# szcompressor/sz

Measured on AMD Instinct MI355X. Metric: compression GB/s (input), 512^3 float32 ABS 1e-4, higher is better.
Workload: dtype f32

## Files before the change

### sz_amd/csrc/szh_fittile.h

```cpp
#pragma once

namespace szh_ft {
constexpr int BMAX = 7;
constexpr int LPR = 1;
template <class T> struct shape {
    static constexpr int VT = 16 / (int)sizeof(T);
    static constexpr int SEGB = sizeof(T) == 4 ? 32 : 16;
    static constexpr int WIDTH = SEGB * BMAX + 2 * VT;
    static constexpr int PITCH = WIDTH + VT;
    static constexpr int BUF = BMAX * PITCH;
    static_assert((WIDTH + VT - 1) / VT <= 64 * LPR && PITCH % VT == 0, "row pieces per lane");
};
template <class T> inline bool applies(const szh_geom3 &G, const void *base)
{
    if (G.ndim != 3) return false;
    if (G.g0.early > BMAX || G.g1.early > BMAX || G.g2.early > BMAX) return false;
    if (G.g0.count < 2 || G.g1.count < 2 || G.g2.count < 2) return false;
    if ((G.g2.count % shape<T>::VT) != 0 || ((uintptr_t)base & 15) != 0) return false;
    return (double)G.g0.num * G.g1.num * ((G.g2.num + shape<T>::SEGB - 1) / shape<T>::SEGB) < 2.0e9;
}
}

template <class T>
__global__ __launch_bounds__(64) void k_fit_tile(szh_geom3 G, const T *__restrict__ data, T *coef, uint8_t *blk_lor, T noise, int use_mean, T mean, u64 *minmax, int nseg)
{
    using namespace szh_ft;
    typedef shape<T> S;
    constexpr int VT = S::VT;
    __shared__ __attribute__((aligned(16))) T buf[2][S::BUF];
    const int lane = (int)threadIdx.x;
    const int col = (int)(blockIdx.x / (unsigned)nseg), segi = (int)(blockIdx.x - (unsigned)col * (unsigned)nseg);
    const int b0 = col / G.g1.num, b1 = col - b0 * G.g1.num;
    const int s0 = szh_blk_size(G.g0, b0), s1 = szh_blk_size(G.g1, b1), o0 = szh_blk_start(G.g0, b0), o1 = szh_blk_start(G.g1, b1);
    const int bkbeg = segi * S::SEGB, bkend = bkbeg + S::SEGB < G.g2.num ? bkbeg + S::SEGB : G.g2.num;
    const int kbeg = szh_blk_start(G.g2, bkbeg), kend = bkend < G.g2.num ? szh_blk_start(G.g2, bkend) : G.g2.count;
    const int ka = kbeg / VT * VT, kb = (kend + VT - 1) / VT * VT, nvec = (kb - ka) / VT;
    const int b2 = bkbeg + lane;
    const bool has = b2 < bkend;
    const int s2 = has ? szh_blk_size(G.g2, b2) : 1, k0 = has ? szh_blk_start(G.g2, b2) - ka : 0;
    int bs = s0 < s1 ? s0 : s1; if (s2 < bs) bs = s2;

    const T qnan = (T)__builtin_nanf("");
    T vmin = qnan, vmax = qnan;
    uint4 pf[BMAX][LPR];
    auto fetch = [&](int i) {
#pragma unroll
        for (int j = 0; j < BMAX; ++j)
#pragma unroll
            for (int q = 0; q < LPR; ++q) {
                const int v = lane + 64 * q;
                pf[j][q] = uint4{0u, 0u, 0u, 0u};
                if (j < s1 && v < nvec) pf[j][q] = *reinterpret_cast<const uint4 *>(data + (int64_t)(o0 + i) * G.d0 + (int64_t)(o1 + j) * G.d1 + ka + v * VT);
            }
    };
    auto place = [&](int w) {
#pragma unroll
        for (int j = 0; j < BMAX; ++j)
#pragma unroll
            for (int q = 0; q < LPR; ++q) {
                const int v = lane + 64 * q;
                if (j < s1 && v < nvec) {
                    *reinterpret_cast<uint4 *>(&buf[w][j * S::PITCH + v * VT]) = pf[j][q];
                    T x[VT]; __builtin_memcpy(x, &pf[j][q], 16);
                    const int e_lo = kbeg - (ka + v * VT), e_hi = kend - (ka + v * VT);
#pragma unroll
                    for (int e = 0; e < VT; ++e) {
                        const T xv = (e >= e_lo && e < e_hi) ? x[e] : qnan;
                        vmin = sizeof(T) == 8 ? (T)__builtin_fmin((double)vmin, (double)xv) : (T)__builtin_fminf((float)vmin, (float)xv);
                        vmax = sizeof(T) == 8 ? (T)__builtin_fmax((double)vmax, (double)xv) : (T)__builtin_fmaxf((float)vmax, (float)xv);
                    }
                }
            }
    };
    fetch(0);
    T fx = 0, fy = 0, fz = 0, f = 0, err_sz = 0;
    T xs[4 * (BMAX - 1)];
#pragma unroll
    for (int e = 0; e < 4 * (BMAX - 1); ++e) xs[e] = 0;
#pragma unroll
    for (int i = 0; i < BMAX; ++i) {
        if (i >= s0) break;
        const int w = i & 1;
        place(w);
        __syncthreads();
        if (i + 1 < s0) fetch(i + 1);
        if (has) {
            const T *P = &buf[w][k0], *Q = &buf[w ^ 1][k0];
            T sum_x = 0;
#pragma unroll
            for (int j = 0; j < BMAX; ++j) {
                if (j < s1) {
                    T row[BMAX];
#pragma unroll
                    for (int k = 0; k < BMAX; ++k) row[k] = k < s2 ? P[j * S::PITCH + k] : (T)0;
                    T sum_y = 0;
#pragma unroll
                    for (int k = 0; k < BMAX; ++k) if (k < s2) { const T c = row[k]; sum_y += c; fz += c * (T)k; }
                    fy += sum_y * (T)j;
                    sum_x += sum_y;
                }
            }
            fx += sum_x * (T)i;
            f += sum_x;
            if (i >= 1 && i < bs) {
                const int bmi = bs - i;
#pragma unroll
                for (int q = 0; q < 4; ++q) {
                    const int j = (q & 2) ? bmi : i, k = (q & 1) ? bmi : i;
                    const T x = P[j * S::PITCH + k];
                    const T psz = P[j * S::PITCH + k - 1] + P[(j - 1) * S::PITCH + k] + Q[j * S::PITCH + k] - P[(j - 1) * S::PITCH + k - 1] - Q[j * S::PITCH + k - 1]
                                  - Q[(j - 1) * S::PITCH + k] + Q[(j - 1) * S::PITCH + k - 1];
                    const T e1 = szh_abs(psz - x) + noise;
                    if (use_mean) { const T e2 = szh_abs(mean - x); err_sz += (e1 < e2 ? e1 : e2); }
                    else err_sz += e1;
                    xs[(i - 1) * 4 + q] = x;
                }
            }
        }
        __syncthreads();
    }
    if (has) {
        const T coeff = (T)(1.0 / (double)((int64_t)s0 * s1 * s2));
        const T a = ((T)2 * fx / (T)(s0 - 1) - f) * (T)6 * coeff / (T)(s0 + 1);
        const T b = ((T)2 * fy / (T)(s1 - 1) - f) * (T)6 * coeff / (T)(s1 + 1);
        const T c = ((T)2 * fz / (T)(s2 - 1) - f) * (T)6 * coeff / (T)(s2 + 1);
        const T d = f * coeff - ((T)(s0 - 1) * a / (T)2 + (T)(s1 - 1) * b / (T)2 + (T)(s2 - 1) * c / (T)2);
        T err_reg = 0;
#pragma unroll
        for (int i = 1; i < BMAX; ++i) {
            if (i < bs) {
                const int bmi = bs - i;
#pragma unroll
                for (int q = 0; q < 4; ++q) {
                    const int j = (q & 2) ? bmi : i, k = (q & 1) ? bmi : i;
                    const T preg = a * (T)i + b * (T)j + c * (T)k + d;
                    err_reg += szh_abs(preg - xs[(i - 1) * 4 + q]);
                }
            }
        }
        const int64_t blk = ((int64_t)b0 * G.g1.num + b1) * G.g2.num + b2;
        coef[blk] = a; coef[G.nblocks + blk] = b; coef[2 * G.nblocks + blk] = c; coef[3 * G.nblocks + blk] = d;
        blk_lor[blk] = err_reg < err_sz ? 0 : 1;
    }
    u64 lmin = vmin == vmin ? ord_enc(vmin) : ~0ull, lmax = vmax == vmax ? ord_enc(vmax) : 0ull;
    lmin = wave_min_u64(lmin); lmax = wave_max_u64(lmax);
    if (lane == 0) {
        if (lmin < *(volatile u64 *)&minmax[0]) atomicMin(&minmax[0], lmin);
        if (lmax > *(volatile u64 *)&minmax[1]) atomicMax(&minmax[1], lmax);
    }
}
```

### sz_amd/csrc/szhip_kernels.h

```cpp
#pragma once
#include <hip/hip_runtime.h>
#include "szh_core.h"
#include "szh_pencil.h"
#include "szh_bufio.h"

typedef unsigned long long u64;

#ifdef SZH_HIPSIM
#define SZH_DYN_SMEM(name) char *name = hipsim_dyn_smem()
#else
#define SZH_DYN_SMEM(name) extern __shared__ __attribute__((aligned(16))) char name[]
#endif

__device__ __forceinline__ u64 ord_enc(float v)
{
    unsigned u = __float_as_uint(v);
    u = (u & 0x80000000u) ? ~u : (u | 0x80000000u);
    return (u64)u;
}
__device__ __forceinline__ u64 ord_enc(double v)
{
    u64 u = (u64)__double_as_longlong(v);
    u = (u & 0x8000000000000000ull) ? ~u : (u | 0x8000000000000000ull);
    return u;
// ... 211 lines not shown
        } else if (w == NP) szh_tile_store<T, B>(a, TI, TJ, L);
        else szh_tile_fill<T, B>(a, TI, TJ, L);
        if (!a.persist) break;
    }
}

template <class T> struct GlobAcc {
    const T *p; int64_t d0, d1;
    __device__ T operator()(int i, int j, int k) const { return p[i * d0 + j * d1 + k]; }
    __device__ T operator()(int j, int k) const { return p[j * d1 + k]; }
};

template <class T>
__global__ __launch_bounds__(256) void k_fit_select(szh_geom3 G, const T *__restrict__ data, T *coef, uint8_t *blk_lor,
                                                    T noise, int use_mean, T mean, u64 *minmax)
{
    __shared__ u64 red[8];
    const int lane = threadIdx.x & 63, wid = threadIdx.x >> 6;
    const int64_t b = (int64_t)blockIdx.x * 256 + threadIdx.x;
    u64 lmin = ~0ull, lmax = 0ull;
    if (b < G.nblocks) {
        const int nb2 = G.g2.num, nb1 = G.g1.num;
        const int b2 = (int)(b % nb2);
        const int64_t c = b / nb2;
        const int b1 = (int)(c % nb1), b0 = (int)(c / nb1);
        const int s0 = szh_blk_size(G.g0, b0), s1 = szh_blk_size(G.g1, b1), s2 = szh_blk_size(G.g2, b2);
        const GlobAcc<T> A{data + (int64_t)szh_blk_start(G.g0, b0) * G.d0 + (int64_t)szh_blk_start(G.g1, b1) * G.d1 + szh_blk_start(G.g2, b2),
                           G.d0, G.d1};
        T c4[4];
        auto range = [&](T v) { const u64 oe = ord_enc(v); const bool num = v == v; lmin = num && oe < lmin ? oe : lmin; lmax = num && oe > lmax ? oe : lmax; };
        int reg;
        if (G.ndim == 2) {
            c4[0] = 0;
            szh_fit_block_2d<T>(A, s1, s2, c4 + 1, range);
            reg = szh_select_block_2d<T>(A, s1, s2, c4 + 1, noise);
        } else {
            szh_fit_block<T>(A, s0, s1, s2, c4, range);
            reg = szh_select_block<T>(A, s0, s1, s2, c4, noise, use_mean, mean);
        }
        for (int e = 0; e < 4; ++e) coef[(int64_t)e * G.nblocks + b] = c4[e];
        blk_lor[b] = reg ? 0 : 1;
    }
    lmin = wave_min_u64(lmin); lmax = wave_max_u64(lmax);
    if (lane == 0) { red[wid] = lmin; red[4 + wid] = lmax; }
    __syncthreads();
    if (threadIdx.x == 0) {
        u64 mn = red[0], mx = red[4];
        for (int w = 1; w < 4; ++w) { mn = red[w] < mn ? red[w] : mn; mx = red[4 + w] > mx ? red[4 + w] : mx; }
        atomicMin(&minmax[0], mn); atomicMax(&minmax[1], mx);
    }
}

template <class T>
__global__ __launch_bounds__(256) void k_minmax(const T *__restrict__ data, int64_t n, u64 *minmax)
{
    __shared__ u64 red[8];
    u64 lmin = ~0ull, lmax = 0ull;
    for (int64_t i = (int64_t)blockIdx.x * 256 + threadIdx.x; i < n; i += (int64_t)gridDim.x * 256) {
        const T v = data[i]; const u64 e = ord_enc(v); const bool num = v == v;
        lmin = num && e < lmin ? e : lmin; lmax = num && e > lmax ? e : lmax;
    }
    lmin = wave_min_u64(lmin); lmax = wave_max_u64(lmax);
    if ((threadIdx.x & 63) == 0) { red[threadIdx.x >> 6] = lmin; red[4 + (threadIdx.x >> 6)] = lmax; }
    __syncthreads();
    if (threadIdx.x == 0) {
        u64 mn = red[0], mx = red[4];
        for (int w = 1; w < 4; ++w) { mn = red[w] < mn ? red[w] : mn; mx = red[4 + w] > mx ? red[4 + w] : mx; }
        atomicMin(&minmax[0], mn); atomicMax(&minmax[1], mx);
    }
}

template <class T>
__global__ __launch_bounds__(256) void k_gather_mean(const T *__restrict__ data, szh_meanwalk w, int64_t count, T *out)
{
    const int64_t m = (int64_t)blockIdx.x * 256 + threadIdx.x;
    if (m < count) out[m] = data[szh_meanwalk_pos(w, m)];
}

#define SZH_LDS_RADIUS_BINS 4096
template <class T, bool FREQ>
__device__ __forceinline__ void sample_body(szh_geom3 G, const T *__restrict__ data, int64_t nrows, int sd, double ebD, T mean,
                                            unsigned max_radius, unsigned *radius_hist, unsigned *freq_hist, u64 *within)
{
    __shared__ unsigned sh_r[SZH_LDS_RADIUS_BINS];
    __shared__ unsigned sh_f[FREQ ? 8192 : 1];
    for (int i = threadIdx.x; i < SZH_LDS_RADIUS_BINS; i += 256) sh_r[i] = 0;
    if (FREQ) for (int i = threadIdx.x; i < 8192; i += 256) sh_f[i] = 0;
    __syncthreads();
    const int64_t rpp = G.g1.count - 1, r2 = G.g2.count;
    const bool two_d = G.ndim == 2;
    unsigned w = 0;
    for (int64_t ridx = (int64_t)blockIdx.x * 256 + threadIdx.x; ridx < nrows; ridx += (int64_t)gridDim.x * 256) {
        const int64_t n1 = two_d ? 0 : ridx / rpp + 1, n2 = two_d ? ridx + 1 : ridx - (n1 - 1) * rpp + 1;
        const int64_t c0 = two_d ? szh_sample_col0_2d(n2, sd) : sd - ((n1 + n2) % sd);
        const int64_t origin = n1 * G.d0 + n2 * r2;
        for (int64_t m = 0;; ++m) {
            const int64_t col = c0 + m * sd;
            if (m > 0 && col >= r2) break;
            const int64_t pos = origin + col;
            if (pos >= G.n) break;
            unsigned ri; int fi, we;
            szh_sample_point<T>(data, pos, r2, two_d ? 0 : G.d0, ebD, mean, max_radius, &ri, &fi, &we);
            if (ri < SZH_LDS_RADIUS_BINS) atomicAdd(&sh_r[ri], 1u); else atomicAdd(&radius_hist[ri], 1u);
            if (FREQ) atomicAdd(&sh_f[fi], 1u);
            w += (unsigned)we;
        }
    }
    w = wave_sum_u32(w);
    if ((threadIdx.x & 63) == 0 && w) atomicAdd(within, (u64)w);
    __syncthreads();
    for (int i = threadIdx.x; i < SZH_LDS_RADIUS_BINS; i += 256) if (sh_r[i]) atomicAdd(&radius_hist[i], sh_r[i]);
    if (FREQ) for (int i = threadIdx.x; i < 8192; i += 256) if (sh_f[i]) atomicAdd(&freq_hist[i], sh_f[i]);
}
template <class T, bool FREQ>
__global__ __launch_bounds__(256) void k_sample(szh_geom3 G, const T *__restrict__ data, int64_t nrows, int sd, double ebD, T mean,
                                                unsigned max_radius, unsigned *radius_hist, unsigned *freq_hist, u64 *within)
{
    sample_body<T, FREQ>(G, data, nrows, sd, ebD, mean, max_radius, radius_hist, freq_hist, within);
}
template <class T, bool FREQ>
__global__ void k_sample_walk(szh_geom3 G, const T *__restrict__ data, int sd, double ebD, T mean, unsigned max_radius, unsigned *radius_hist,
                              unsigned *freq_hist, u64 *within)
{
    if (threadIdx.x != 0 || blockIdx.x != 0) return;
    const int64_t r3 = G.g2.count, r2 = G.g1.count, r23 = r2 * r3, len = G.n;
    int64_t oc = sd - 2, n1 = 1, n2 = 1, pos = r23 + r3 + oc;
    u64 w = 0;
    while (pos < len) {
        unsigned ri; int fi, we;
        szh_sample_point<T>(data, pos, r3, r23, ebD, mean, max_radius, &ri, &fi, &we);
        atomicAdd(&radius_hist[ri], 1u);
        if (FREQ) atomicAdd(&freq_hist[fi], 1u);
        w += (unsigned)we;
        oc += sd;
        if (oc >= r3) {
            n2++;
            if (n2 == r2) { n1++; n2 = 1; pos += r3; }
            const int64_t oc2 = (n1 + n2) % sd;
            pos += (r3 + sd - oc) + (sd - oc2);
            oc = sd - oc2;
            if (oc == 0) oc++;
        } else pos += sd;
    }
    if (w) atomicAdd(within, w);
}

template <class T>
__device__ __forceinline__ void sample_view_body(const unsigned tid, szh_geom3 G, const T *data, int64_t p0, int64_t p1, int64_t nrows, int sd, double ebD,
                                                 unsigned max_radius, unsigned *radius_hist, u64 *within)
{
    __shared__ unsigned sh_r[SZH_LDS_RADIUS_BINS];
    for (int i = tid; i < SZH_LDS_RADIUS_BINS; i += 256) sh_r[i] = 0;
    __syncthreads();
    const int64_t rpp = G.g1.count - 1, r2 = G.g2.count;
    unsigned w = 0;
    for (int64_t ridx = (int64_t)blockIdx.x * 256 + tid; ridx < nrows; ridx += (int64_t)gridDim.x * 256) {
        const int64_t n1 = ridx / rpp + 1, n2 = ridx - (n1 - 1) * rpp + 1;
        const int64_t c0 = sd - ((n1 + n2) % sd);
        const int64_t origin = n1 * G.d0 + n2 * r2;
        for (int64_t m = 0;; ++m) {
            const int64_t col = c0 + m * sd;
            if (m > 0 && col >= r2) break;
            const int64_t pos = origin + col;
            if (pos >= G.n) break;
            unsigned ri; int fi, we;
            if (col < r2) szh_sample_point<T>(data, n1 * p0 + n2 * p1 + col, p1, p0, ebD, (T)0, max_radius, &ri, &fi, &we);
            else szh_sample_point_view<T>(data, pos, r2, G.d0, p0, p1, ebD, max_radius, &ri, &we);
            if (ri < SZH_LDS_RADIUS_BINS) atomicAdd(&sh_r[ri], 1u); else atomicAdd(&radius_hist[ri], 1u);
            w += (unsigned)we;
        }
    }
    w = wave_sum_u32(w);
    if ((tid & 63) == 0 && w) atomicAdd(within, (u64)w);
    __syncthreads();
    for (int i = tid; i < SZH_LDS_RADIUS_BINS; i += 256) if (sh_r[i]) atomicAdd(&radius_hist[i], sh_r[i]);
}
template <class T>
__global__ __launch_bounds__(256) void k_sample_view(szh_geom3 G, const T *__restrict__ data, int64_t p0, int64_t p1, int64_t nrows, int sd, double ebD,
                                                     unsigned max_radius, unsigned *radius_hist, u64 *within)
{
    __shared__ unsigned sh_r[SZH_LDS_RADIUS_BINS];
    for (int i = threadIdx.x; i < SZH_LDS_RADIUS_BINS; i += 256) sh_r[i] = 0;
    __syncthreads();
    const int64_t rpp = G.g1.count - 1, r2 = G.g2.count;
    unsigned w = 0;
    for (int64_t ridx = (int64_t)blockIdx.x * 256 + threadIdx.x; ridx < nrows; ridx += (int64_t)gridDim.x * 256) {
        const int64_t n1 = ridx / rpp + 1, n2 = ridx - (n1 - 1) * rpp + 1;
        const int64_t c0 = sd - ((n1 + n2) % sd);
        const int64_t origin = n1 * G.d0 + n2 * r2;
        for (int64_t m = 0;; ++m) {
            const int64_t col = c0 + m * sd;
            if (m > 0 && col >= r2) break;
            const int64_t pos = origin + col;
            if (pos >= G.n) break;
            unsigned ri; int fi, we;
// ... 1157 lines not shown
```

### sz_amd/csrc/szhip_sz21.inc

```
static bool book_declines(unsigned rec_status, unsigned long long plan_status, int test_switch) { return rec_status != 0 || plan_status != 0 || test_switch != 0; }

struct sz21_plan {
    bool use_beam = false;
    bool segenc = false;
    bool seghist = false;
    bool dev_book = false;
    bool sliced = false;
    int slices_req = 1;
    int se_vw = 1, se_segb = 0, se_nseg = 0, se_nrmax = szh_se::NR; size_t se_tile = 0;
    int sh_rshift = 0;
    bool revise(unsigned enc_maxlen) { if (!segenc || enc_maxlen <= 32) return false; segenc = false; seghist = false; return true; }
};
template <class T>
sz21_plan sz21_make_plan(const szhip_ctx *ctx, const szh_geom3 &G, unsigned intervals, size_t reg_count, bool beam_ok, bool overlap, bool feed, size_t meta_len)
{
    sz21_plan P;
    const int64_t n = G.n;
    P.use_beam = !overlap && beam_ok;
    const int segenc_sw = tune_int("SZ_HIP_SEGENC", 1);
    P.segenc = G.ndim == 3 && segenc_sw != 0 && (!feed || segenc_sw == 2);
    P.se_vw = (G.g2.count % 8) == 0 ? 8 : ((G.g2.count % 4) == 0 ? 4 : 1);
    if (P.segenc) {
        bool ok = intervals < 65536 && (double)n < 4.0e9;
        if ((int64_t)G.g0.late * G.g1.late * G.g2.late < 32) ok = false;
        const size_t fixed = ((size_t)intervals + 1) * 8 + 16 + szh_se::seg_window_words(G, 32) * 4 + 64;
        const size_t lds_cap = (size_t)63 * 1024, want = (size_t)std::max(4, tune_int("SZ_HIP_SEG_TILE_KB", 14)) * 1024;
        if (ok && fixed + szh_se::seg_tile_bytes(G, 1, P.se_vw) > lds_cap) ok = false;
        if (ok) {
            const size_t budget = std::min(lds_cap - fixed, std::max(want, szh_se::seg_tile_bytes(G, 1, P.se_vw)));
            int sb = 1;
            while (sb < G.g2.num && szh_se::seg_tile_bytes(G, sb + 1, P.se_vw) <= budget && szh_se::seg_pieces_per_thread(G, sb + 1, P.se_vw) <= (size_t)szh_se::PF) ++sb;
            sb = (G.g2.num + (G.g2.num + sb - 1) / sb - 1) / ((G.g2.num + sb - 1) / sb);
            if (const int f = tune_int("SZ_HIP_SEG_SEGB", 0)) sb = std::max(1, std::min(f, sb));
            P.se_segb = sb;
            P.se_nseg = (G.g2.num + sb - 1) / sb;
            P.se_tile = szh_se::seg_tile_bytes(G, sb, P.se_vw);
            const int rows_typ = (2 * G.g0.split > G.g0.num ? G.g0.early : G.g0.late) * (2 * G.g1.split > G.g1.num ? G.g1.early : G.g1.late);
            const int runs_typ = std::max(1, sb * rows_typ), rounds_typ = (runs_typ + 256 * szh_se::NR - 1) / (256 * szh_se::NR);
            P.se_nrmax = std::max(1, std::min(szh_se::NR, (runs_typ + 256 * rounds_typ - 1) / (256 * rounds_typ)));
            if ((double)G.g0.num * G.g1.num >= 2.0e9) ok = false;
        }
        P.segenc = ok;
    }
    P.seghist = P.segenc && intervals <= SZH_COL_HBINS && tune_int("SZ_HIP_SEGHIST", 1) != 0;
    if (P.seghist) P.sh_rshift = hist_rshift(intervals, 4096);
    P.dev_book = P.segenc && reg_count == 0 && !ctx->no_dev_book && tune_int("SZ_HIP_DEV_BOOK", 0) != 0 && G.g0.num * G.g1.num <= 1024 * SZH_COL_SCAN_PER &&
                 tune_int("SZ_HIP_SEG_SCAN1", 1) != 0 && meta_len + 8 + 4 + sizeof(T) + 1 + sizeof(T) <= 3072;
    P.slices_req = tune_int("SZ_HIP_SLICES", ctx->gate ? tune_int("SZ_HIP_SLICES_POOL", 2) : 4);
    P.sliced = P.use_beam && P.slices_req > 1 && !P.seghist;
    return P;
}

template <class T>
struct sz21_call : call_base {
    static constexpr int is_double = sizeof(T) == 8;
    static constexpr int64_t LINE = 128 / (int64_t)sizeof(T);
    const szhip_params *const prm; const unsigned char *meta; const size_t meta_len; const int out_on_device; unsigned char **const out; size_t *const out_size;
    const double eb_in; const T eb;
    const bool two_d;
    const szh_geom3 G; const int ncoef, ncols; const int64_t n, nb;
    const int tp_on = tune_int("SZ_HIP_TIMING", 0); double tp_t[32]; const char *tp_n[32]; int tp_k = 0;
    const T *d_in = nullptr; u64 *sm = nullptr; T *d_coef = nullptr; uint8_t *d_lor = nullptr; uint16_t *d_nat = nullptr, *d_blk = nullptr; unsigned *d_hist = nullptr, *h_hist = nullptr;
    T noise = 0; bool fit_tile = false; int ft_nseg = 0;
    size_t ind_bytes = 0; unsigned char *ind_bits = nullptr; u64 *nreg_h = nullptr, *minmax_h = nullptr;
    unsigned intervals = 0; int use_mean = 0; T mean = 0; size_t reg_count = 0;
    std::vector<unsigned char> meta_own;
    sz21_plan P;
    unsigned *tile_done = nullptr; size_t beam_words = 0;
    int perm_segb = 1, perm_nseg = 1; size_t perm_lds = 0;
    std::vector<szh_se::seg_t> se_segs; std::vector<u64> tab_code; std::vector<uint8_t> tab_len;
    unsigned enc_maxlen = 0; bool enc32 = false; size_t lds_e32 = 0;
    unsigned char *hdr = nullptr; size_t pre_len = 0, sections_total = 0, hdr_len = 0, unpred_bytes = 0, total_len = 0; u64 total_bits = 0, total_unpred = 0;
    u64 h_small[SM_COUNT];
    szhost_coeffs cf;
    size_t sec_len[4] = {0, 0, 0, 0};
    std::vector<std::thread> section_threads;
    std::atomic<int> section_failed{0};
    std::vector<unsigned char> all_reg_keep;
    std::vector<uint32_t> blk_of_rank;
    size_t chain_done[4] = {0, 0, 0, 0};
    size_t chain_avail = 0;
    double chain_t0[4] = {0, 0, 0, 0}, chain_t1[4] = {0, 0, 0, 0};
    bool overlap = false, feed = false, two_pieces = false;
    fed_call_guard fed_guard;
    T *hcoef = nullptr;
    bool pool_busy = false;
    bool cf_own = false;
    sz21_call(szhip_ctx *c, size_t r0, size_t r1, size_t r2, double eb_, const szhip_params *p, const unsigned char *m, size_t ml, int ood, unsigned char **o, size_t *os)
        : call_base(c), prm(p), meta(m), meta_len(ml), out_on_device(ood), out(o), out_size(os), eb_in(eb_), eb((T)eb_), two_d(r0 == 0),
          G(r0 == 0 ? szh_make_geom2((int)r1, (int)r2) : szh_make_geom3((int)r0, (int)r1, (int)r2)), ncoef(r0 == 0 ? 3 : 4), ncols(G.g0.num * G.g1.num), n(G.n), nb(G.nblocks)
    {
        memset(&cf, 0, sizeof(cf));
        S.n_elements = (uint64_t)n; S.n_blocks = (uint64_t)nb;
    }
    ~sz21_call() {
        join_sections();
        if (ctx->chain_pool) ctx->chain_pool->disarm();
        if (cf_own) for (int e = 0; e < 4; ++e) { cf.codes[e] = nullptr; cf.unpred[e] = nullptr; }
        szhost_coeffs_free(&cf);
    }
    void join_sections() {
        for (auto &x : section_threads) if (x.joinable()) x.join();
        if (pool_busy && ctx->chain_pool) { ctx->chain_pool->wait_all(); pool_busy = false; }
    }
    void TP(const char *nm) { if (tp_on && tp_k < 32) { tp_t[tp_k] = now_ms() - t_begin; tp_n[tp_k++] = nm; } }
    void print_trace() const { if (tp_on) { for (int i = 0; i < tp_k; ++i) fprintf(stderr, "%s %.2f | ", tp_n[i], tp_t[i]); fprintf(stderr, "\n"); } }
    bool is_lorenzo(int64_t bb) const { return (ind_bits[bb >> 3] >> (7 - (bb & 7))) & 1; }
    size_t count_lorenzo(int64_t bb, int64_t b_end) const {
        size_t ones = 0;
        for (; bb < b_end && (bb & 7); ++bb) ones += is_lorenzo(bb);
        for (; bb + 64 <= b_end; bb += 64) { uint64_t w8; memcpy(&w8, ind_bits + (bb >> 3), 8); ones += (size_t)__builtin_popcountll(w8); }
        for (; bb < b_end; ++bb) ones += is_lorenzo(bb);
        return ones;
    }
    size_t chains_done() const {
        size_t p = reg_count;
        for (int e = 0; e < ncoef; ++e) { const size_t d = __atomic_load_n(&chain_done[e], __ATOMIC_ACQUIRE); if (d < p) p = d; }
        return p;
    }
    int launch_fit(hipStream_t s_, int um, T mn) {
        if (fit_tile) hipLaunchKernelGGL((k_fit_tile<T>), dim3((unsigned)((int64_t)ncols * ft_nseg)), dim3(64), 0, s_, G, d_in, d_coef, d_lor, noise, um, mn, sm + SM_MINMAX, ft_nseg);
        else hipLaunchKernelGGL((k_fit_select<T>), dim3((unsigned)((nb + 255) / 256)), dim3(256), 0, s_, G, d_in, d_coef, d_lor, noise, um, mn, sm + SM_MINMAX);
        HIPCHK(hipGetLastError());
        return SZHIP_OK;
    }
    int launch_pack_lor(hipStream_t s_) {
        hipLaunchKernelGGL(k_pack_lor, dim3((unsigned)((ind_bytes + 255) / 256)), dim3(256), 0, s_, (const uint8_t *)d_lor, nb, (uint8_t *)ctx->lor_bits.p, sm + SM_NREG);
        HIPCHK(hipGetLastError());
        HIPCHK(hipMemcpyAsync(ind_bits, ctx->lor_bits.p, ind_bytes, hipMemcpyDeviceToHost, s_));
        HIPCHK(hipMemcpyAsync(nreg_h, sm + SM_NREG, 8, hipMemcpyDeviceToHost, s_));
        return SZHIP_OK;
    }
    int stage_and_fit(const void *data, int data_on_device) {
        TRY(stage_input(ctx, data, data_on_device, (size_t)n, &d_in));
        TRY(clear_small(ctx, &sm));
        static const u64 minmax_init[2] = {~0ull, 0ull};
        HIPCHK(hipMemcpyAsync(sm + SM_MINMAX, minmax_init, 16, hipMemcpyHostToDevice, st));
        TRY(ensure(ctx, ctx->coef, (size_t)nb * 4 * sizeof(T)));
        TRY(ensure(ctx, ctx->blk_lor, (size_t)nb));
        d_coef = (T *)ctx->coef.p;
        d_lor = (uint8_t *)ctx->blk_lor.p;
        HIPCHK(hipEventRecord(ctx->ev[0], st));
        TP("ev0");
        HIPCHK(hipEventRecord(ctx->ev_in, st));
        HIPCHK(hipStreamWaitEvent(ctx->stream2, ctx->ev_in, 0));
        noise = (T)((double)eb * (two_d ? 0.81 : 1.22));
        fit_tile = !two_d && szh_ft::applies<T>(G, d_in) && tune_int("SZ_HIP_FIT_TILE", 0) != 0;
        ft_nseg = (G.g2.num + szh_ft::shape<T>::SEGB - 1) / szh_ft::shape<T>::SEGB;
        TRY(launch_fit(ctx->stream2, 0, (T)0));
        ind_bytes = ((size_t)nb + 7) / 8;
        TRY(ensure(ctx, ctx->lor_bits, ind_bytes + 8));
        TRY(ensure_pinned2(ctx, ind_bytes + 32));
        ind_bits = (unsigned char *)ctx->pinned2 + 32;
        nreg_h = (u64 *)ctx->pinned2;
        minmax_h = (u64 *)ctx->pinned2 + 2;
        TRY(launch_pack_lor(ctx->stream2));
        HIPCHK(hipMemcpyAsync(minmax_h, sm + SM_MINMAX, 16, hipMemcpyDeviceToHost, ctx->stream2));
        HIPCHK(hipEventRecord(ctx->ev_fit, ctx->stream2));
        return SZHIP_OK;
    }
    int choose_intervals() {
        intervals = prm->quantization_intervals;
        const unsigned max_radius = prm->max_quant_intervals / 2;
        if (intervals == 0) {
            const int64_t md = (int64_t)(int)std::sqrt((double)n);
            const szh_meanwalk w = two_d ? szh_make_meanwalk(n, INT64_MAX / 2, INT64_MAX / 2, md) : szh_make_meanwalk(n, G.d0, G.g2.count, md);
            int64_t M = 0, M_hi = n / std::max<int64_t>(md - 2, 1) + 2;
            while (szh_meanwalk_pos(w, M_hi) < n) M_hi *= 2;
            while (M < M_hi) { int64_t mid = (M + M_hi) / 2; if (szh_meanwalk_pos(w, mid) >= n) M_hi = mid; else M = mid + 1; }
            TRY(ensure(ctx, ctx->samples, (size_t)M * sizeof(T)));
            TRY(ensure_pinned(ctx, std::max<size_t>((size_t)M * sizeof(T), (size_t)(max_radius + 8192) * 4 + 64)));
            hipLaunchKernelGGL((k_gather_mean<T>), dim3((unsigned)((M + 255) / 256)), dim3(256), 0, st, d_in, w, M, (T *)ctx->samples.p);
            HIPCHK(hipGetLastError());
            HIPCHK(hipMemcpyAsync(ctx->pinned, ctx->samples.p, (size_t)M * sizeof(T), hipMemcpyDeviceToHost, st));
            TP("mean enqueued");
            HIPCHK(hipStreamSynchronize(st));
            TP("mean on host");
            double h0 = now_ms();
            const double smean = szhost_seq_mean(is_double, ctx->pinned, (size_t)M);
            host_ms += now_ms() - h0;
            TRY(ensure(ctx, ctx->hist, (size_t)(max_radius + 8192) * 4 + 64));
            unsigned *d_rh = (unsigned *)ctx->hist.p, *d_fh = d_rh + max_radius;
            HIPCHK(hipMemsetAsync(d_rh, 0, (size_t)(max_radius + 8192) * 4, st));
            const int64_t nrows = szh_sample_row_limit(G, prm->sample_distance);
            if (!two_d && (G.g0.count <= 1 || G.g1.count <= 1)) {
                hipLaunchKernelGGL((k_sample_walk<T, true>), dim3(1), dim3(64), 0, st, G, d_in, prm->sample_distance, (double)eb, (T)smean, max_radius, d_rh, d_fh, sm + SM_WITHIN);
                HIPCHK(hipGetLastError());
            } else if (nrows > 0) {
                int grid = (int)std::min<int64_t>((nrows + 255) / 256, 1024);
                hipLaunchKernelGGL((k_sample<T, true>), dim3(grid), dim3(256), 0, st, G, d_in, nrows, prm->sample_distance, (double)eb, (T)smean, max_radius, d_rh, d_fh, sm + SM_WITHIN);
                HIPCHK(hipGetLastError());
            }
            unsigned *s_hist = (unsigned *)ctx->pinned;
            u64 within = 0;
            HIPCHK(hipMemcpyAsync(s_hist, d_rh, (size_t)(max_radius + 8192) * 4, hipMemcpyDeviceToHost, st));
            HIPCHK(hipMemcpyAsync(&within, sm + SM_WITHIN, 8, hipMemcpyDeviceToHost, st));
            TP("sample enqueued");
            HIPCHK(hipStreamSynchronize(st));
            TP("sample on host");
            h0 = now_ms();
            u64 sample_count = 0;
            for (unsigned i = 0; i < max_radius; ++i) sample_count += s_hist[i];
            szhost_decision dec;
            szhost_decide(is_double, s_hist, max_radius, s_hist + max_radius, sample_count, within, prm->pred_threshold, (double)eb, smean, &dec);
            host_ms += now_ms() - h0;
            intervals = dec.intervals; use_mean = two_d ? 0 : dec.use_mean;
            if (use_mean) {
                T *d_sum = (T *)(sm + SM_MEANSUM);
                hipLaunchKernelGGL((k_mean_seq<T>), dim3(1), dim3(64), 0, st, d_in, n, (T)dec.dense_pos, eb, d_sum, sm + SM_MEANCNT);
                HIPCHK(hipGetLastError());
                T hsum = 0; u64 hcnt = 0;
                HIPCHK(hipMemcpyAsync(&hsum, d_sum, sizeof(T), hipMemcpyDeviceToHost, st));
                HIPCHK(hipMemcpyAsync(&hcnt, sm + SM_MEANCNT, 8, hipMemcpyDeviceToHost, st));
                HIPCHK(hipStreamSynchronize(st));
                if (hcnt > 0) mean = hsum / (T)hcnt;
            }
        }
        if (intervals > 65536 || intervals < 4) FAIL(SZHIP_ERR_UNSUP, "quantization interval count %u outside [4,65536]", intervals);
        S.intervals = intervals; S.use_mean = use_mean;
        return SZHIP_OK;
    }
    int join_fit() {
        HIPCHK(hipStreamWaitEvent(st, ctx->ev_fit, 0));
        if (use_mean) {
            TRY(launch_fit(st, use_mean, mean));
            HIPCHK(hipMemsetAsync(sm + SM_NREG, 0, 8, st));
            TRY(launch_pack_lor(st));
            HIPCHK(hipStreamSynchronize(st));
        } else HIPCHK(hipEventSynchronize(ctx->ev_fit));
        TP("fit joined");
        reg_count = (size_t)*nreg_h;
        S.n_reg_blocks = reg_count;
        if (reg_count == 0 && ctx->chain_pool) ctx->chain_pool->disarm();
        meta_own.assign(meta, meta + meta_len);
        if (prm->flags & SZHIP_RANGE_FROM_DATA) {
            if (meta_len < 4 + 20 + 2 * sizeof(T)) FAIL(SZHIP_ERR_ARG, "parameter bytes too short for a range field");
            const T lo = (T)ord_dec<T>(minmax_h[0]), hi = (T)ord_dec<T>(minmax_h[1]);
            const T range = hi - lo, top = lo + range;
            unsigned char *q = meta_own.data() + 4 + 20;
            if (is_double) { szhost_put_f64be(q, (double)lo); szhost_put_f64be(q + 8, (double)top); }
            else { szhost_put_f32be(q, (float)lo); szhost_put_f32be(q + 4, (float)top); }
            S.vmin = (double)lo; S.vmax = (double)hi;
            if ((double)range <= eb_in) {
                HIPCHK(hipStreamSynchronize(ctx->stream2)); HIPCHK(hipStreamSynchronize(st));
                *out = nullptr; *out_size = 0;
                S.ms_total = now_ms() - t_begin;
                return SZHIP_CONSTANT;
            }
        }
        meta = meta_own.data();
        return SZHIP_OK;
    }
    void make_section(int e) {
        std::vector<uint32_t> h32(65536, 0);
        for (size_t i = 0; i < reg_count; ++i) h32[(size_t)cf.codes[e][i]]++;
        const huff_ptr ch(szhost_huff_build(131072, h32.data(), nullptr, 65536));
        if (!ch) { section_failed = 1; return; }
        const size_t tb = szhost_huff_tree_size(ch.get());
        const size_t enc_cap = (size_t)((ch->total_bits + 7) / 8) + 16;
        if (sizeof(T) + 12 + tb + 8 + enc_cap + 4 + cf.unpred_count[e] * sizeof(T) > ctx->sec_pin_cap[e]) { section_failed = 1; return; }
        unsigned char *const sec0 = ctx->sec_pin[e];
        unsigned char *q = sec0;
        if (is_double) szhost_put_f64be(q, cf.prec[e]); else szhost_put_f32be(q, (float)cf.prec[e]);
        q += sizeof(T);
        szhost_put_u32be(q, 32768); q += 4;
        szhost_put_u32be(q, (uint32_t)tb); q += 4;
        szhost_put_u32be(q, (uint32_t)ch->n_nodes); q += 4;
        szhost_huff_tree_write(ch.get(), q); q += tb;
        const size_t enc = szhost_huff_encode_i32(ch.get(), cf.codes[e], reg_count, q + 8);
        szhost_put_u64be(q, enc); q += 8 + enc;
        szhost_put_u32be(q, (uint32_t)cf.unpred_count[e]); q += 4;
        memcpy(q, cf.unpred[e], cf.unpred_count[e] * sizeof(T)); q += cf.unpred_count[e] * sizeof(T);
        sec_len[e] = (size_t)(q - sec0);
    }
    int prepare_chains() {
        for (int e = 0; e < ncoef; ++e) {
            const size_t bound = sizeof(T) + 12 + (13 * 2 * std::min<size_t>(reg_count, 65536) + 16) + 8 + (8 * reg_count + 16) + 4 + reg_count * sizeof(T) + 64;
            if (ctx->sec_pin_cap[e] < bound) {
                HIPCHK(hipStreamSynchronize(ctx->stream2)); HIPCHK(hipStreamSynchronize(st));
                if (ctx->sec_pin[e]) { HIPCHK(hipHostFree(ctx->sec_pin[e])); ctx->sec_pin[e] = nullptr; ctx->sec_pin_cap[e] = 0; }
                HIPCHK(hipHostMalloc((void **)&ctx->sec_pin[e], bound + bound / 8, hipHostMallocDefault));
                ctx->sec_pin_cap[e] = bound + bound / 8;
            }
        }
        TRY(ensure(ctx, ctx->reg_flags, (size_t)nb * 8));
        TRY(ensure(ctx, ctx->reg_rank, (size_t)nb * 8));
        TRY(ensure(ctx, ctx->coef_compact, reg_count * 4 * sizeof(T)));
        hipLaunchKernelGGL(k_reg_flags, dim3((unsigned)((nb + 255) / 256)), dim3(256), 0, st, (const uint8_t *)d_lor, nb, (u64 *)ctx->reg_flags.p);
        TRY(scan_u64(ctx, (const u64 *)ctx->reg_flags.p, nb, (u64 *)ctx->reg_rank.p, sm + SM_SCRATCH));
        hipLaunchKernelGGL((k_move_coef<T, 0>), dim3((unsigned)((nb + 255) / 256)), dim3(256), 0, st, (const uint8_t *)d_lor, (const u64 *)ctx->reg_rank.p, nb, (int64_t)reg_count, d_coef, (T *)ctx->coef_compact.p);
        HIPCHK(hipGetLastError());
#ifndef SZH_SYNC_LAUNCH
        overlap = !beam_applies<T>(G, d_in, reg_count) && !two_d && !ctx->gate && !ctx->no_chain_overlap && g_compress_calls.load() <= 1;
        if (overlap) { TRY(probe_streams(ctx)); overlap = ctx->streams_independent == 1; }
#endif
        feed = beam_applies<T>(G, d_in, reg_count) && !ctx->gate && !ctx->no_chain_overlap && g_compress_calls.load() <= 1 && tune_int("SZ_HIP_BEAM_FEED", 1) &&
               G.g0.num >= 2 && reg_count >= (size_t)tune_int("SZ_HIP_FEED_MIN_REG", 65536);
#ifndef SZH_SYNC_LAUNCH
        feed = feed && (G.d0 % 128) == 0;
        if (feed) { TRY(probe_streams(ctx)); feed = ctx->streams_independent == 1; }
#endif
        if (feed) feed = fed_guard.try_raise();
        TRY(ensure_pinned3(ctx, reg_count * 4 * sizeof(T) + (overlap ? ((size_t)nb + 64) * 4 * sizeof(T) + 256 : 0)));
        hcoef = (T *)ctx->pinned3;
        return SZHIP_OK;
    }
    int run_chains() {
        chain_avail = reg_count;
        struct AvailAll {
// ... 941 lines not shown
```

Baseline: 377.7.

## Add one-thread-per-block register fit kernel and rework sampling histograms

Adds a new fit kernel, k_fit_wide, where each thread fits one full 3D block from registers. It uses a statically unrolled sliding-window pass over rows and fuses the regression/Lorenzo choice, bit packing and region counting into the same kernel, so the separate pack_lor launch is skipped. It is enabled by default for float. The sampling kernel now packs two 16-bit frequency counters per LDS word with periodic flushes, uses fewer LDS radius bins, and sizes its grid from the CU count. The histogram memset is also moved earlier to overlap with the mean gather. The fully unrolled 49-step body risks high register pressure and low occupancy.

```diff
diff --git a/sz_amd/csrc/szh_fittile.h b/sz_amd/csrc/szh_fittile.h
--- a/sz_amd/csrc/szh_fittile.h
+++ b/sz_amd/csrc/szh_fittile.h
@@ -1,4 +1,5 @@
 #pragma once
+#include <utility>
 
 namespace szh_ft {
 constexpr int BMAX = 7;
@@ -149,3 +150,209 @@
         if (lmax > *(volatile u64 *)&minmax[1]) atomicMax(&minmax[1], lmax);
     }
 }
+
+#ifdef SZH_HIPSIM
+#define SZH_FW_STEP_FENCE() ((void)0)
+#define SZH_FW_PIN(p) ((void)0)
+#else
+#define SZH_FW_STEP_FENCE() __builtin_amdgcn_sched_barrier(0)
+#define SZH_FW_PIN(p) asm volatile("" : "+v"(p))
+#endif
+namespace szh_fw {
+template <class T> struct shape {
+    static constexpr int VT = 16 / (int)sizeof(T);
+    static constexpr int NP = (szh_ft::BMAX + 2 * (VT - 1)) / VT;
+    static constexpr int DEPTH = 1;
+};
+template <class F, int... Is>
+__device__ __forceinline__ void static_steps(F &&f, std::integer_sequence<int, Is...>) { (f(std::integral_constant<int, Is>{}), ...); }
+template <class T>
+__device__ __forceinline__ void block_pass(const szh_geom3 &G, const T *__restrict__ base, int off, int np, int s0, int s1, int s2, T noise, int use_mean, T mean,
+                                           T (&c4)[4], int &reg, T &vmin, T &vmax)
+{
+    constexpr int B = szh_ft::BMAX, VT = shape<T>::VT, NP = shape<T>::NP, D = shape<T>::DEPTH, STEPS = B * B;
+    int bs = s0 < s1 ? s0 : s1; if (s2 < bs) bs = s2;
+    const int d = B - bs;
+    const T qnan = (T)__builtin_nanf("");
+    uint4 buf[D][NP];
+    auto fetch = [&](int slot, int i, int j) {
+        int64_t ro = (int64_t)i * G.d0 + (int64_t)j * G.d1;
+        SZH_FW_PIN(ro);
+        const T *rp = base + ro;
+#pragma unroll
+        for (int q = 0; q < NP; ++q) {
+            const T *p = rp + q * VT;
+            const bool there = i < B - 1 && j < B - 1 ? (q < 2 || q < np) : (i < s0 && j < s1 && q < np);
+            buf[slot][q] = *reinterpret_cast<const uint4 *>(there ? p : base);
+        }
+    };
+    auto pick = [&](const T (&row)[B], int C) -> T {
+        const T a = C >= 0 && C < B ? row[C < 0 ? 0 : (C < B ? C : B - 1)] : (T)0, a1 = C >= 1 && C <= B ? row[C < 1 ? 0 : (C <= B ? C - 1 : B - 1)] : (T)0;
+        return d ? a1 : a;
+    };
+    T fx = 0, fy = 0, fz = 0, f = 0, err_sz = 0, sum_x = 0;
+    T xs[4 * (B - 1)];
+#pragma unroll
+    for (int e = 0; e < 4 * (B - 1); ++e) xs[e] = 0;
+    T Q[4][4], N[4][4], ppc[4], er[4], xv[4];
+#pragma unroll
+    for (int r = 0; r < 4; ++r) {
+        ppc[r] = 0; er[r] = 0; xv[r] = 0;
+#pragma unroll
+        for (int c = 0; c < 4; ++c) { Q[r][c] = 0; N[r][c] = 0; }
+    }
+#pragma unroll
+    for (int t = 0; t < D; ++t) fetch(t, t / B, t % B);
+    static_steps([&](auto tc) {
+        constexpr int t = decltype(tc)::value;
+        constexpr int i = t / B, j = t % B, slot = t % D;
+        T win[NP * VT];
+        __builtin_memcpy(win, buf[slot], sizeof(win));
+        if (t + D < STEPS) fetch(slot, (t + D) / B, (t + D) % B);
+        SZH_FW_STEP_FENCE();
+#pragma unroll
+        for (int s = 1; s < VT; s <<= 1)
+#pragma unroll
+            for (int k = 0; k + s < NP * VT; ++k) win[k] = (off & s) ? win[k + s] : win[k];
+        T row[B];
+#pragma unroll
+        for (int k = 0; k < B; ++k) row[k] = win[k];
+        const bool act = i < s0 && j < s1;
+        if (j == 0) sum_x = 0;
+        T sum_y = 0;
+#pragma unroll
+        for (int k = 0; k < B; ++k) {
+            const bool on = (i < B - 1 && j < B - 1 && k < B - 1) || (act && k < s2);
+            const T c = row[k], cn = on ? c : qnan;
+            sum_y = on ? sum_y + c : sum_y; fz = on ? fz + c * (T)k : fz;
+            vmin = sizeof(T) == 8 ? (T)__builtin_fmin((double)vmin, (double)cn) : (T)__builtin_fminf((float)vmin, (float)cn);
+            vmax = sizeof(T) == 8 ? (T)__builtin_fmax((double)vmax, (double)cn) : (T)__builtin_fmaxf((float)vmax, (float)cn);
+        }
+        const bool act_r = (i < B - 1 && j < B - 1) || act, act_p = i < B - 1 || i < s0;
+        fy = act_r ? fy + sum_y * (T)j : fy; sum_x = act_r ? sum_x + sum_y : sum_x;
+        if (j == B - 1) { fx = act_p ? fx + sum_x * (T)i : fx; f = act_p ? f + sum_x : f; }
+        const int c1 = B - i - d, c0 = c1 - 1;
+        T pc[4];
+        pc[0] = i >= 1 ? row[i >= 1 ? i - 1 : 0] : (T)0; pc[1] = row[i]; pc[2] = pick(row, B - i - 1); pc[3] = pick(row, B - i);
+        if (i + 1 < B) {
+            const T nc[4] = {pc[1], row[i + 1 < B ? i + 1 : B - 1], pick(row, B - i - 2), pc[2]};
+#pragma unroll
+            for (int c = 0; c < 4; ++c) {
+                if (j == i) N[0][c] = nc[c];
+                if (j == i + 1) N[1][c] = nc[c];
+                if (j == B - i - 2 || j == B - i - 3) N[2][c] = (j == c0 - 1) ? nc[c] : N[2][c];
+                if (j == B - i - 1 || j == B - i - 2) N[3][c] = (j == c0) ? nc[c] : N[3][c];
+            }
+        }
+        if (i >= 1 && j >= 1) {
+            auto stencil = [&](const T (&Qj)[4], const T (&Qm)[4], int ck) -> T {
+                const T psz = pc[ck - 1] + ppc[ck] + Qj[ck] - ppc[ck - 1] - Qj[ck - 1] - Qm[ck] + Qm[ck - 1];
+                const T e1 = szh_abs(psz - pc[ck]) + noise;
+                const T e2 = szh_abs(mean - pc[ck]);
+                return (use_mean && e1 >= e2) ? e2 : e1;
+            };
+            if (j == i) { er[0] = stencil(Q[1], Q[0], 1); er[1] = stencil(Q[1], Q[0], 3); xv[0] = pc[1]; xv[1] = pc[3]; }
+            if (j <= B - i && j >= B - i - 1) {
+                const T e2 = stencil(Q[3], Q[2], 1), e3 = stencil(Q[3], Q[2], 3);
+                const bool far = j == c1;
+                er[2] = far ? e2 : er[2]; er[3] = far ? e3 : er[3]; xv[2] = far ? pc[1] : xv[2]; xv[3] = far ? pc[3] : xv[3];
+            }
+        }
+#pragma unroll
+        for (int c = 0; c < 4; ++c) ppc[c] = pc[c];
+        SZH_FW_PIN(fz); SZH_FW_PIN(fy); SZH_FW_PIN(sum_x); SZH_FW_PIN(vmin); SZH_FW_PIN(vmax);
+#pragma unroll
+        for (int c = 0; c < 4; ++c) { SZH_FW_PIN(ppc[c]); SZH_FW_PIN(N[0][c]); SZH_FW_PIN(N[1][c]); SZH_FW_PIN(N[2][c]); SZH_FW_PIN(N[3][c]); SZH_FW_PIN(er[c]); SZH_FW_PIN(xv[c]); }
+        if (j == B - 1) {
+            if (i >= 1) {
+#pragma unroll
+                for (int q = 0; q < 4; ++q) { err_sz = i < bs ? err_sz + er[q] : err_sz; xs[(i >= 1 ? i - 1 : 0) * 4 + q] = xv[q]; }
+            }
+#pragma unroll
+            for (int r = 0; r < 4; ++r)
+#pragma unroll
+                for (int c = 0; c < 4; ++c) Q[r][c] = N[r][c];
+        }
+    }, std::make_integer_sequence<int, STEPS>{});
+    const T coeff = (T)(1.0 / (double)((int64_t)s0 * s1 * s2));
+    const T a = ((T)2 * fx / (T)(s0 - 1) - f) * (T)6 * coeff / (T)(s0 + 1);
+    const T b = ((T)2 * fy / (T)(s1 - 1) - f) * (T)6 * coeff / (T)(s1 + 1);
+    const T c = ((T)2 * fz / (T)(s2 - 1) - f) * (T)6 * coeff / (T)(s2 + 1);
+    const T dd = f * coeff - ((T)(s0 - 1) * a / (T)2 + (T)(s1 - 1) * b / (T)2 + (T)(s2 - 1) * c / (T)2);
+    T err_reg = 0;
+#pragma unroll
+    for (int i = 1; i < B; ++i) {
+        if (i < bs) {
+            const int bmi = bs - i;
+#pragma unroll
+            for (int q = 0; q < 4; ++q) {
+                const int j = (q & 2) ? bmi : i, k = (q & 1) ? bmi : i;
+                const T preg = a * (T)i + b * (T)j + c * (T)k + dd;
+                err_reg += szh_abs(preg - xs[(i - 1) * 4 + q]);
+            }
+        }
+    }
+    c4[0] = a; c4[1] = b; c4[2] = c; c4[3] = dd;
+    reg = err_reg < err_sz ? 1 : 0;
+}
+}
+
+template <class T>
+__global__ __launch_bounds__(256) void k_fit_wide(szh_geom3 G, const T *__restrict__ data, T *coef, uint8_t *blk_lor, uint8_t *bits, u64 *n_reg, T noise, int use_mean,
+                                                  T mean, u64 *minmax)
+{
+    constexpr int VT = szh_fw::shape<T>::VT;
+    __shared__ u64 red[8];
+    const int lane = threadIdx.x & 63, wid = threadIdx.x >> 6;
+    const int64_t b = (int64_t)blockIdx.x * 256 + threadIdx.x;
+    const bool has = b < G.nblocks;
+    int s0 = 0, s1 = 0, s2 = 0, off = 0, np = 0;
+    const T *base = data;
+    if (has) {
+        const int nb2 = G.g2.num, nb1 = G.g1.num;
+        const int b2 = (int)(b % nb2);
+        const int64_t c = b / nb2;
+        const int b1 = (int)(c % nb1), b0 = (int)(c / nb1);
+        s0 = szh_blk_size(G.g0, b0); s1 = szh_blk_size(G.g1, b1); s2 = szh_blk_size(G.g2, b2);
+        const int k0 = szh_blk_start(G.g2, b2);
+        off = k0 & (VT - 1);
+        np = (off + s2 + VT - 1) / VT;
+        base = data + (int64_t)szh_blk_start(G.g0, b0) * G.d0 + (int64_t)szh_blk_start(G.g1, b1) * G.d1 + (k0 - off);
+    }
+    int bs = s0 < s1 ? s0 : s1; if (s2 < bs) bs = s2;
+    T c4[4] = {0, 0, 0, 0};
+    int reg = 0;
+    u64 lmin = ~0ull, lmax = 0ull;
+    if (__all(has && bs >= szh_ft::BMAX - 1)) {
+        const T qnan = (T)__builtin_nanf("");
+        T vmin = qnan, vmax = qnan;
+        szh_fw::block_pass<T>(G, base, off, np, s0, s1, s2, noise, use_mean, mean, c4, reg, vmin, vmax);
+        if (vmin == vmin) lmin = ord_enc(vmin);
+        if (vmax == vmax) lmax = ord_enc(vmax);
+    } else if (has) {
+        const GlobAcc<T> A{base + off, G.d0, G.d1};
+        auto range = [&](T v) { const u64 oe = ord_enc(v); const bool num = v == v; lmin = num && oe < lmin ? oe : lmin; lmax = num && oe > lmax ? oe : lmax; };
+        szh_fit_block<T>(A, s0, s1, s2, c4, range);
+        reg = szh_select_block<T>(A, s0, s1, s2, c4, noise, use_mean, mean);
+    }
+    if (has) {
+        for (int e = 0; e < 4; ++e) coef[(int64_t)e * G.nblocks + b] = c4[e];
+        blk_lor[b] = reg ? 0 : 1;
+    }
+    const unsigned long long lor = __ballot(has && !reg ? 1 : 0);
+    if (lane < 8 && b - lane + 8 * lane < G.nblocks) {
+        unsigned v = (unsigned)(lor >> (8 * lane)) & 0xffu;
+        v = ((v & 0xf0u) >> 4) | ((v & 0x0fu) << 4); v = ((v & 0xccu) >> 2) | ((v & 0x33u) << 2); v = ((v & 0xaau) >> 1) | ((v & 0x55u) << 1);
+        bits[((b - lane) >> 3) + lane] = (uint8_t)v;
+    }
+    const unsigned long long regs = __ballot(has && reg ? 1 : 0);
+    if (lane == 0 && regs) atomicAdd(n_reg, (u64)__popcll(regs));
+    lmin = wave_min_u64(lmin); lmax = wave_max_u64(lmax);
+    if (lane == 0) { red[wid] = lmin; red[4 + wid] = lmax; }
+    __syncthreads();
+    if (threadIdx.x == 0) {
+        u64 mn = red[0], mx = red[4];
+        for (int w = 1; w < 4; ++w) { mn = red[w] < mn ? red[w] : mn; mx = red[4 + w] > mx ? red[4 + w] : mx; }
+        atomicMin(&minmax[0], mn); atomicMax(&minmax[1], mx);
+    }
+}
diff --git a/sz_amd/csrc/szhip_kernels.h b/sz_amd/csrc/szhip_kernels.h
--- a/sz_amd/csrc/szhip_kernels.h
+++ b/sz_amd/csrc/szhip_kernels.h
@@ -317,15 +317,33 @@
 __device__ __forceinline__ void sample_body(szh_geom3 G, const T *__restrict__ data, int64_t nrows, int sd, double ebD, T mean,
                                             unsigned max_radius, unsigned *radius_hist, unsigned *freq_hist, u64 *within)
 {
-    __shared__ unsigned sh_r[SZH_LDS_RADIUS_BINS];
-    __shared__ unsigned sh_f[FREQ ? 8192 : 1];
-    for (int i = threadIdx.x; i < SZH_LDS_RADIUS_BINS; i += 256) sh_r[i] = 0;
-    if (FREQ) for (int i = threadIdx.x; i < 8192; i += 256) sh_f[i] = 0;
+    constexpr int RBINS = FREQ ? 1024 : SZH_LDS_RADIUS_BINS;
+    __shared__ unsigned sh_r[RBINS];
+    __shared__ unsigned sh_f[FREQ ? 4096 : 1];
+    for (int i = threadIdx.x; i < RBINS; i += 256) sh_r[i] = 0;
+    if (FREQ) for (int i = threadIdx.x; i < 4096; i += 256) sh_f[i] = 0;
     __syncthreads();
     const int64_t rpp = G.g1.count - 1, r2 = G.g2.count;
     const bool two_d = G.ndim == 2;
+    const int64_t per_trip = 256 * ((r2 + sd - 1) / sd + 1);
+    const bool direct = FREQ && per_trip > 65535;
+    auto flush_f = [&]() {
+        for (int i = threadIdx.x; i < 4096; i += 256) {
+            const unsigned v = sh_f[i];
+            if (v & 0xffffu) atomicAdd(&freq_hist[2 * i], v & 0xffffu);
+            if (v >> 16) atomicAdd(&freq_hist[2 * i + 1], v >> 16);
+            sh_f[i] = 0;
+        }
+    };
     unsigned w = 0;
-    for (int64_t ridx = (int64_t)blockIdx.x * 256 + threadIdx.x; ridx < nrows; ridx += (int64_t)gridDim.x * 256) {
+    int64_t pending = 0;
+    for (int64_t r0 = (int64_t)blockIdx.x * 256; r0 < nrows; r0 += (int64_t)gridDim.x * 256) {
+        if (FREQ && !direct) {
+            if (pending + per_trip > 65535) { __syncthreads(); flush_f(); __syncthreads(); pending = 0; }
+            pending += per_trip;
+        }
+        const int64_t ridx = r0 + threadIdx.x;
+        if (ridx >= nrows) continue;
         const int64_t n1 = two_d ? 0 : ridx / rpp + 1, n2 = two_d ? ridx + 1 : ridx - (n1 - 1) * rpp + 1;
         const int64_t c0 = two_d ? szh_sample_col0_2d(n2, sd) : sd - ((n1 + n2) % sd);
         const int64_t origin = n1 * G.d0 + n2 * r2;
@@ -336,16 +354,16 @@
             if (pos >= G.n) break;
             unsigned ri; int fi, we;
             szh_sample_point<T>(data, pos, r2, two_d ? 0 : G.d0, ebD, mean, max_radius, &ri, &fi, &we);
-            if (ri < SZH_LDS_RADIUS_BINS) atomicAdd(&sh_r[ri], 1u); else atomicAdd(&radius_hist[ri], 1u);
-            if (FREQ) atomicAdd(&sh_f[fi], 1u);
+            if (ri < (unsigned)RBINS) atomicAdd(&sh_r[ri], 1u); else atomicAdd(&radius_hist[ri], 1u);
+            if (FREQ) { if (direct) atomicAdd(&freq_hist[fi], 1u); else atomicAdd(&sh_f[fi >> 1], (fi & 1) ? 0x10000u : 1u); }
             w += (unsigned)we;
         }
     }
     w = wave_sum_u32(w);
     if ((threadIdx.x & 63) == 0 && w) atomicAdd(within, (u64)w);
     __syncthreads();
-    for (int i = threadIdx.x; i < SZH_LDS_RADIUS_BINS; i += 256) if (sh_r[i]) atomicAdd(&radius_hist[i], sh_r[i]);
-    if (FREQ) for (int i = threadIdx.x; i < 8192; i += 256) if (sh_f[i]) atomicAdd(&freq_hist[i], sh_f[i]);
+    for (int i = threadIdx.x; i < RBINS; i += 256) if (sh_r[i]) atomicAdd(&radius_hist[i], sh_r[i]);
+    if (FREQ && !direct) flush_f();
 }
 template <class T, bool FREQ>
 __global__ __launch_bounds__(256) void k_sample(szh_geom3 G, const T *__restrict__ data, int64_t nrows, int sd, double ebD, T mean,
diff --git a/sz_amd/csrc/szhip_sz21.inc b/sz_amd/csrc/szhip_sz21.inc
--- a/sz_amd/csrc/szhip_sz21.inc
+++ b/sz_amd/csrc/szhip_sz21.inc
@@ -61,7 +61,7 @@
     const szh_geom3 G; const int ncoef, ncols; const int64_t n, nb;
     const int tp_on = tune_int("SZ_HIP_TIMING", 0); double tp_t[32]; const char *tp_n[32]; int tp_k = 0;
     const T *d_in = nullptr; u64 *sm = nullptr; T *d_coef = nullptr; uint8_t *d_lor = nullptr; uint16_t *d_nat = nullptr, *d_blk = nullptr; unsigned *d_hist = nullptr, *h_hist = nullptr;
-    T noise = 0; bool fit_tile = false; int ft_nseg = 0;
+    T noise = 0; bool fit_tile = false, fit_wide = false; int ft_nseg = 0;
     size_t ind_bytes = 0; unsigned char *ind_bits = nullptr; u64 *nreg_h = nullptr, *minmax_h = nullptr;
     unsigned intervals = 0; int use_mean = 0; T mean = 0; size_t reg_count = 0;
     std::vector<unsigned char> meta_own;
@@ -120,13 +120,16 @@
     }
     int launch_fit(hipStream_t s_, int um, T mn) {
         if (fit_tile) hipLaunchKernelGGL((k_fit_tile<T>), dim3((unsigned)((int64_t)ncols * ft_nseg)), dim3(64), 0, s_, G, d_in, d_coef, d_lor, noise, um, mn, sm + SM_MINMAX, ft_nseg);
+        else if (fit_wide) hipLaunchKernelGGL((k_fit_wide<T>), dim3((unsigned)((nb + 255) / 256)), dim3(256), 0, s_, G, d_in, d_coef, d_lor, (uint8_t *)ctx->lor_bits.p, sm + SM_NREG, noise, um, mn, sm + SM_MINMAX);
         else hipLaunchKernelGGL((k_fit_select<T>), dim3((unsigned)((nb + 255) / 256)), dim3(256), 0, s_, G, d_in, d_coef, d_lor, noise, um, mn, sm + SM_MINMAX);
         HIPCHK(hipGetLastError());
         return SZHIP_OK;
     }
     int launch_pack_lor(hipStream_t s_) {
-        hipLaunchKernelGGL(k_pack_lor, dim3((unsigned)((ind_bytes + 255) / 256)), dim3(256), 0, s_, (const uint8_t *)d_lor, nb, (uint8_t *)ctx->lor_bits.p, sm + SM_NREG);
-        HIPCHK(hipGetLastError());
+        if (!fit_wide) {
+            hipLaunchKernelGGL(k_pack_lor, dim3((unsigned)((ind_bytes + 255) / 256)), dim3(256), 0, s_, (const uint8_t *)d_lor, nb, (uint8_t *)ctx->lor_bits.p, sm + SM_NREG);
+            HIPCHK(hipGetLastError());
+        }
         HIPCHK(hipMemcpyAsync(ind_bits, ctx->lor_bits.p, ind_bytes, hipMemcpyDeviceToHost, s_));
         HIPCHK(hipMemcpyAsync(nreg_h, sm + SM_NREG, 8, hipMemcpyDeviceToHost, s_));
         return SZHIP_OK;
@@ -147,13 +150,15 @@
         noise = (T)((double)eb * (two_d ? 0.81 : 1.22));
         fit_tile = !two_d && szh_ft::applies<T>(G, d_in) && tune_int("SZ_HIP_FIT_TILE", 0) != 0;
         ft_nseg = (G.g2.num + szh_ft::shape<T>::SEGB - 1) / szh_ft::shape<T>::SEGB;
-        TRY(launch_fit(ctx->stream2, 0, (T)0));
+        const int fit_wide_sw = tune_int("SZ_HIP_FIT_WIDE", 1);
+        fit_wide = !fit_tile && !two_d && szh_ft::applies<T>(G, d_in) && (fit_wide_sw >= 2 || (fit_wide_sw == 1 && !is_double));
         ind_bytes = ((size_t)nb + 7) / 8;
         TRY(ensure(ctx, ctx->lor_bits, ind_bytes + 8));
         TRY(ensure_pinned2(ctx, ind_bytes + 32));
         ind_bits = (unsigned char *)ctx->pinned2 + 32;
         nreg_h = (u64 *)ctx->pinned2;
         minmax_h = (u64 *)ctx->pinned2 + 2;
+        TRY(launch_fit(ctx->stream2, 0, (T)0));
         TRY(launch_pack_lor(ctx->stream2));
         HIPCHK(hipMemcpyAsync(minmax_h, sm + SM_MINMAX, 16, hipMemcpyDeviceToHost, ctx->stream2));
         HIPCHK(hipEventRecord(ctx->ev_fit, ctx->stream2));
@@ -170,6 +175,9 @@
             while (M < M_hi) { int64_t mid = (M + M_hi) / 2; if (szh_meanwalk_pos(w, mid) >= n) M_hi = mid; else M = mid + 1; }
             TRY(ensure(ctx, ctx->samples, (size_t)M * sizeof(T)));
             TRY(ensure_pinned(ctx, std::max<size_t>((size_t)M * sizeof(T), (size_t)(max_radius + 8192) * 4 + 64)));
+            TRY(ensure(ctx, ctx->hist, (size_t)(max_radius + 8192) * 4 + 64));
+            unsigned *d_rh = (unsigned *)ctx->hist.p, *d_fh = d_rh + max_radius;
+            HIPCHK(hipMemsetAsync(d_rh, 0, (size_t)(max_radius + 8192) * 4, st));
             hipLaunchKernelGGL((k_gather_mean<T>), dim3((unsigned)((M + 255) / 256)), dim3(256), 0, st, d_in, w, M, (T *)ctx->samples.p);
             HIPCHK(hipGetLastError());
             HIPCHK(hipMemcpyAsync(ctx->pinned, ctx->samples.p, (size_t)M * sizeof(T), hipMemcpyDeviceToHost, st));
@@ -179,15 +187,13 @@
             double h0 = now_ms();
             const double smean = szhost_seq_mean(is_double, ctx->pinned, (size_t)M);
             host_ms += now_ms() - h0;
-            TRY(ensure(ctx, ctx->hist, (size_t)(max_radius + 8192) * 4 + 64));
-            unsigned *d_rh = (unsigned *)ctx->hist.p, *d_fh = d_rh + max_radius;
-            HIPCHK(hipMemsetAsync(d_rh, 0, (size_t)(max_radius + 8192) * 4, st));
             const int64_t nrows = szh_sample_row_limit(G, prm->sample_distance);
             if (!two_d && (G.g0.count <= 1 || G.g1.count <= 1)) {
                 hipLaunchKernelGGL((k_sample_walk<T, true>), dim3(1), dim3(64), 0, st, G, d_in, prm->sample_distance, (double)eb, (T)smean, max_radius, d_rh, d_fh, sm + SM_WITHIN);
                 HIPCHK(hipGetLastError());
             } else if (nrows > 0) {
-                int grid = (int)std::min<int64_t>((nrows + 255) / 256, 1024);
+                int grid = (int)std::min<int64_t>((nrows + 255) / 256, (int64_t)8 * ctx->cus);
+                if (const int g = tune_int("SZ_HIP_SAMPLE_GRID", 0)) grid = std::max(1, std::min(g, grid));
                 hipLaunchKernelGGL((k_sample<T, true>), dim3(grid), dim3(256), 0, st, G, d_in, nrows, prm->sample_distance, (double)eb, (T)smean, max_radius, d_rh, d_fh, sm + SM_WITHIN);
                 HIPCHK(hipGetLastError());
             }
@@ -223,8 +229,8 @@
     int join_fit() {
         HIPCHK(hipStreamWaitEvent(st, ctx->ev_fit, 0));
         if (use_mean) {
+            HIPCHK(hipMemsetAsync(sm + SM_NREG, 0, 8, st));
             TRY(launch_fit(st, use_mean, mean));
-            HIPCHK(hipMemsetAsync(sm + SM_NREG, 0, 8, st));
             TRY(launch_pack_lor(st));
             HIPCHK(hipStreamSynchronize(st));
         } else HIPCHK(hipEventSynchronize(ctx->ev_fit));
```

Result: faster. 386.5 (median of 6 runs) (+2.3%).
